# cloneofsimo/paint-with-words-sd

Measured on AMD Instinct MI355X. Metric: 512x512 images/sec (30 steps, CFG) SD1.5+PwW, higher is better.
Workload: dtype bf16

## Files before the change

__graft_entry__.py:

```python
import os
import sys

REPO = os.path.dirname(os.path.abspath(__file__))
PKG = os.path.join(REPO, "paint-with-words-sd_amd")
for p in (PKG, REPO, os.path.join(REPO, "tests")):
    if p not in sys.path:
        sys.path.insert(0, p)


def build():
    import build as pww_build
    lib = pww_build.build_lib(verbose=False)
    exe = pww_build.build_native_check()
    import pww_hip
    import paint_with_words
    handle = pww_hip.load_library()
    missing = [n for n in pww_hip.EXPORTS if not hasattr(handle, n)]
    assert not missing, "libpww_hip.so lacks %s" % missing
    from pww_hip import _lib
    built = [(lib, handle.pww_version())]
    for name, build_one in zip(pww_build.SIDE_LIBS, (pww_build.build_long, pww_build.build_scope, pww_build.build_linear, pww_build.build_regions)):
        path = build_one()
        side = _lib.load_side(name)
        assert side is not None, "%s was not built" % path
        missing = [n for n in _lib.SIDE[name]["exports"] if not hasattr(side, n)]
        assert not missing, "%s lacks %s" % (os.path.basename(path), missing)
        built.append((path, getattr(side, "pww_%s_version" % name)()))
    print("built %s and %s" % (", ".join("%s (ABI %d)" % b for b in built), exe))


def smoke():
    import math
    import numpy as np
    import torch
    import pww_hip
    from oracle import pww_oracle as O
    import pww_cases as cases

    assert torch.cuda.is_available(), "smoke() needs a HIP device"
    dev = torch.device("cuda:0")
    print("device arch:", pww_hip.device_arch())

    case = cases.make_attention_case("sd15_n1024")
    dtype = torch.float16
    mod = case["attn_cross"].to(dev, dtype)
    hidden = case["hidden"].to(dev, dtype)
    wf = lambda w, sigma, qk: 0.4 * w * math.log(1 + sigma) * qk.max()
    ctx = {"CONTEXT_TENSOR": case["ctx"].to(dev, dtype), "CROSS_ATTENTION_WEIGHT_1024": case["w"].to(dev),
           "SIGMA": torch.tensor(7.84), "WEIGHT_FUNCTION": wf}
    y = pww_hip.inj_forward(mod, hidden, ctx).float().cpu()
    mod_ref = case["attn_cross"].to("cpu", dtype).float()
    ctx_ref = {"CONTEXT_TENSOR": case["ctx"].to(dtype).float(), "CROSS_ATTENTION_WEIGHT_1024": case["w"],
               "SIGMA": torch.tensor(7.84), "WEIGHT_FUNCTION": wf}
    ref = O.inj_forward(mod_ref, case["hidden"].to(dtype).float(), ctx_ref)
    err = (y - ref).abs().max().item() / ref.abs().max().item()
    print("cross-attention + PwW bias: max err / max|O| = %.3e" % err)
    assert err < 5e-3, err

# ... 27 lines not shown
```

paint-with-words-sd_amd/build.py:

```python
import os
import subprocess
import sys

HERE = os.path.dirname(os.path.abspath(__file__))
REPO = os.path.dirname(HERE)
CSRC = os.path.join(HERE, "csrc")
LIB = os.path.join(HERE, "pww_hip", "libpww_hip.so")
LIB_EXPERIMENTS = os.path.join(HERE, "pww_hip", "libpww_hip_experiments.so")
UNITS = [("pww_api.hip", [], ""), ("pww_attn.hip", [], ""), ("pww_cross.hip", [], ""), ("pww_cross_lean.hip", [], ""), ("pww_reduce.hip", [], ""),
         ("pww_mask.hip", [], ""), ("pww_qproj.hip", [], ""), ("pww_norm.hip", [], ""), ("pww_blocks.hip", [], ""), ("pww_conv.hip", [], ""), ("pww_probs.hip", [], ""),
         ("pww_attn_inst.hip", ["-DPWW_INST_F16"], ".f16"), ("pww_attn_inst.hip", ["-DPWW_INST_BF16"], ".bf16"),
         ("pww_cross_inst.hip", ["-DPWW_INST_F16", "-DPWW_INST_NW=2"], ".f16.nw2"), ("pww_cross_inst.hip", ["-DPWW_INST_F16", "-DPWW_INST_NW=4"], ".f16.nw4"),
         ("pww_cross_inst.hip", ["-DPWW_INST_BF16", "-DPWW_INST_NW=2"], ".bf16.nw2"), ("pww_cross_inst.hip", ["-DPWW_INST_BF16", "-DPWW_INST_NW=4"], ".bf16.nw4")]
EXPERIMENT_UNITS = [("pww_cross_out.hip", [], "")]
_ATTN_HEADERS = ["pww_tile.h", "pww_attn_core.h", "pww_cross_tile.h"]
SIDE_FLAGS = ["-fvisibility=hidden"]
SIDE_LIBS = {
    "long": ("pww_long.hip", _ATTN_HEADERS, "the long-prompt launches"),
    "scope": ("pww_scope.hip", _ATTN_HEADERS, "cross-attention with per-head / per-row score statistics"),
    "linear": ("pww_linear.hip", [], "linear layers with a bias / residual / GEGLU epilogue"),
    "regions": ("pww_regions.hip", [], "region masks and the per-pixel blend of the noise predictions"),
}
SOURCES = sorted({u[0] for u in UNITS + EXPERIMENT_UNITS})
HEADERS = ["pww_common.h", "pww_tile.h", "pww_attn_core.h", "pww_attn_kernel.h", "pww_cross_tile.h", "pww_cross_kernel.h", os.path.join(REPO, "include", "pww_hip.h")]
LIB_LONG, LIB_SCOPE, LIB_LINEAR, LIB_REGIONS = (os.path.join(HERE, "pww_hip", "libpww_hip_%s.so" % n) for n in SIDE_LIBS)
LONG_UNITS, SCOPE_UNITS, LINEAR_UNITS, REGIONS_UNITS = ([(v[0], SIDE_FLAGS, "")] for v in SIDE_LIBS.values())
HIPCC = os.environ.get("HIPCC", "/opt/rocm/bin/hipcc")
FLAGS = ["--offload-arch=gfx950", "-O3", "-std=c++17", "-fPIC", "-Wall",
         "-Wno-unused-function", "-mllvm", "-amdgpu-kernarg-preload-count=16"]


PER_FILE_FLAGS = {"pww_mask.hip": ["-ffp-contract=off"], "pww_regions.hip": ["-ffp-contract=off"]}


def _newer(target, deps):
    if not os.path.exists(target):
        return True
    t = os.path.getmtime(target)
    return any(os.path.getmtime(d) > t for d in deps)


def _deps():
    return ([os.path.join(CSRC, s) for s in SOURCES] + [h if os.path.isabs(h) else os.path.join(CSRC, h) for h in HEADERS] + [__file__])


def _build(lib, units, defines, objdir, verbose, jobs=None):
    os.makedirs(objdir, exist_ok=True)
    order = sorted(units, key=lambda u: {"pww_cross_inst.hip": 0, "pww_attn_inst.hip": 1, "pww_cross_lean.hip": 2}.get(u[0], 3))
    jobs = jobs or max(2, min(len(order), os.cpu_count() or 4, int(os.environ.get("MAX_JOBS", 16))))
    pending, running, objs = list(order), [], []
    while pending or running:
        while pending and len(running) < jobs:
            src, defs, suffix = pending.pop(0)
            o = os.path.join(objdir, src + suffix + ".o")
            objs.append(o)
            cmd = [HIPCC] + FLAGS + defines + defs + PER_FILE_FLAGS.get(src, []) + ["-c", os.path.join(CSRC, src), "-o", o]
            if verbose:
                print(" ".join(cmd))
            running.append((cmd, subprocess.Popen(cmd, stdout=subprocess.PIPE, stderr=subprocess.STDOUT, text=True)))
# ... 4 lines not shown
                q.kill()
            raise RuntimeError("hipcc failed: %s\n%s" % (" ".join(cmd), out))
        if verbose and out.strip():
            print(out)
    subprocess.run([HIPCC, "--offload-arch=gfx950", "-shared", "-fPIC", "-s"] + sorted(objs) + ["-o", lib], check=True)
    return lib


def build_lib(force=False, verbose=False):
    if not force and not _newer(LIB, _deps()):
        return LIB
    return _build(LIB, UNITS, [], os.path.join(HERE, "build"), verbose)


def build_experiments(force=False, verbose=False):
    if not force and not _newer(LIB_EXPERIMENTS, _deps()):
        return LIB_EXPERIMENTS
    return _build(LIB_EXPERIMENTS, UNITS + EXPERIMENT_UNITS, ["-DPWW_EXPERIMENTS=1"], os.path.join(HERE, "build", "experiments"), verbose)


def build_side(name, force=False, verbose=False):
    unit, headers, _ = SIDE_LIBS[name]
    lib = os.path.join(HERE, "pww_hip", "libpww_hip_%s.so" % name)
    deps = [os.path.join(CSRC, f) for f in [unit, "pww_common.h", "pww_side_host.h"] + headers] + [os.path.join(REPO, "include", h) for h in ("pww_hip.h", "pww_hip_%s.h" % name)] + [__file__]
    if not force and not _newer(lib, deps):
        return lib
    return _build(lib, [(unit, SIDE_FLAGS, "")], [], os.path.join(HERE, "build", name), verbose)


def build_long(force=False, verbose=False): return build_side("long", force, verbose)
def build_scope(force=False, verbose=False): return build_side("scope", force, verbose)
def build_linear(force=False, verbose=False): return build_side("linear", force, verbose)
def build_regions(force=False, verbose=False): return build_side("regions", force, verbose)


def _build_check(exe, lib, libname, defines, force):
    src = os.path.join(REPO, "tests", "native", "attn_check.cpp")
    if not force and not _newer(exe, [src, lib, os.path.join(REPO, "include", "pww_hip.h")]):
        return exe
    cmd = [HIPCC, "--offload-arch=gfx950", "-O2", "-std=c++17"] + defines + [src, "-o", exe, "-L" + os.path.dirname(lib), "-l" + libname,
                                                                              "-Wl,-rpath,$ORIGIN/../../paint-with-words-sd_amd/pww_hip"]
    subprocess.run(cmd, check=True)
    return exe


def build_native_check(force=False):
    return _build_check(os.path.join(REPO, "tests", "native", "attn_check"), build_lib(), "pww_hip", [], force)


def build_native_check_experiments(force=False):
    return _build_check(os.path.join(REPO, "tests", "native", "attn_check_experiments"), build_experiments(), "pww_hip_experiments", ["-DPWW_EXPERIMENTS=1"], force)


if __name__ == "__main__":
    force = "--force" in sys.argv
    print(build_lib(force=force, verbose=True))
    print(build_native_check(force=force))
    for name in SIDE_LIBS:
        print(build_side(name, force=force, verbose=True))
    if "--experiments" in sys.argv:
        print(build_experiments(force=force, verbose=True))
        print(build_native_check_experiments(force=force))
```

paint-with-words-sd_amd/pww_hip/_lib.py:

```python
import ctypes
import os

_HERE = os.path.dirname(os.path.abspath(__file__))
LIB_PATH = os.environ.get("PWW_HIP_LIB", os.path.join(_HERE, "libpww_hip.so"))
EXPERIMENTS_LIB_PATH = os.environ.get("PWW_HIP_EXPERIMENTS_LIB", os.path.join(_HERE, "libpww_hip_experiments.so"))

LONG_LIB_PATH = os.environ.get("PWW_HIP_LONG_LIB", os.path.join(_HERE, "libpww_hip_long.so"))
SCOPE_LIB_PATH = os.environ.get("PWW_HIP_SCOPE_LIB", os.path.join(_HERE, "libpww_hip_scope.so"))
LINEAR_LIB_PATH = os.environ.get("PWW_HIP_LINEAR_LIB", os.path.join(_HERE, "libpww_hip_linear.so"))
REGIONS_LIB_PATH = os.environ.get("PWW_HIP_REGIONS_LIB", os.path.join(_HERE, "libpww_hip_regions.so"))

PWW_OK, PWW_EINVAL, PWW_ENOTSUP, PWW_EHIP = 0, -22, -95, -5
MIN_VERSION = 126
DTYPE_F16, DTYPE_BF16 = 0, 1
LAYOUT_NCHW, LAYOUT_NHWC = 0, 1
ACT_NONE, ACT_SILU = 0, 1
LINEAR_NONE, LINEAR_BIAS, LINEAR_BIAS_RESIDUAL, LINEAR_BIAS_GEGLU = 0, 1, 2, 3
MAX_HEAD_DIM = 160

EXPORTS = ("pww_version", "pww_has_experiments", "pww_last_error", "pww_device_arch", "pww_self_attn_fwd", "pww_cross_attn_fwd",
           "pww_cross_attn_fwd_stat", "pww_cross_attn_fwd_stat_ex",
           "pww_qk_reduce", "pww_mask_build", "pww_mask_build_rgb", "pww_mask_build_f32", "pww_resize_tokens", "pww_gauss_blur", "pww_inpaint_prep", "pww_cfg_combine", "pww_store_f32",
           "pww_workspace_bytes", "pww_profile_arm", "pww_profile_elapsed_us", "pww_profile_reset", "pww_debug_timeline", "pww_debug_path_counts",
           "pww_qproj_stat", "pww_qproj_parts", "pww_cross_attn_fwd_parts", "pww_mask_build_f32_levels", "pww_qk_parts", "pww_qk_parts_count",
           "pww_group_norm_fwd", "pww_group_norm_workspace_bytes", "pww_add_layer_norm", "pww_add_layer_norm_bias", "pww_geglu", "pww_bias_residual",
           "pww_conv3x3_workspace_bytes", "pww_conv3x3_fwd", "pww_cross_attn_probs")
EXPERIMENT_EXPORTS = ("pww_cross_attn_fwd_fused", "pww_cross_attn_fwd_fused_ex", "pww_cross_fused_workspace_bytes", "pww_cross_fused_state_bytes",
                      "pww_cross_attn_fwd_parts_out", "pww_cross_attn_out_supported")


LONG_EXPORTS = ("pww_long_version", "pww_long_last_error", "pww_long_qk_parts", "pww_long_qk_parts_count", "pww_long_cross_attn_fwd_parts",
                "pww_long_cross_attn_probs", "pww_long_profile_arm", "pww_long_profile_elapsed_us")
LONG_MIN_VERSION = 100
LONG_MIN_KEYS, LONG_MAX_KEYS = 129, 256


SCOPE_EXPORTS = ("pww_scope_version", "pww_scope_last_error", "pww_scope_head_parts_count", "pww_scope_head_parts", "pww_scope_cross_attn_fwd")
SCOPE_MIN_VERSION = 100
SCOPE_HEAD, SCOPE_ROW = 1, 2


LINEAR_EXPORTS = ("pww_linear_version", "pww_linear_last_error", "pww_linear_workspace_bytes", "pww_linear_fwd")
LINEAR_MIN_VERSION = 100


REGIONS_EXPORTS = ("pww_regions_version", "pww_regions_last_error", "pww_regions_masks", "pww_regions_combine")
REGIONS_MIN_VERSION = 100
REGIONS_MAX, REGIONS_MAX_PLANE, REGIONS_MAX_FEATHER = 8, 9216, 8.0


class AttnDesc(ctypes.Structure):
    _fields_ = [("dtype", ctypes.c_int32), ("B", ctypes.c_int32), ("H", ctypes.c_int32), ("N", ctypes.c_int32),
                ("M", ctypes.c_int32), ("D", ctypes.c_int32),
                ("q_stride", ctypes.c_int64 * 3), ("k_stride", ctypes.c_int64 * 3),
                ("v_stride", ctypes.c_int64 * 3), ("o_stride", ctypes.c_int64 * 3),
                ("scale", ctypes.c_float), ("bias_stride", ctypes.c_int64 * 4)]


class CrossOpts(ctypes.Structure):
    _fields_ = [("size", ctypes.c_uint32), ("bias_cols", ctypes.c_int32), ("coeff_scalar_dev", ctypes.c_void_p),
                ("bias_compact", ctypes.c_void_p), ("col_idx", ctypes.c_void_p), ("R", ctypes.c_int32), ("gated_images", ctypes.c_int32),
                ("compact_stride", ctypes.c_int64 * 2), ("col_idx_stride", ctypes.c_int64)]


class QprojDesc(ctypes.Structure):
    _fields_ = [("dtype", ctypes.c_int32), ("B", ctypes.c_int32), ("N", ctypes.c_int32), ("Cin", ctypes.c_int32), ("H", ctypes.c_int32),
                ("D", ctypes.c_int32), ("M", ctypes.c_int32), ("x_stride", ctypes.c_int64 * 2), ("q_stride", ctypes.c_int64 * 2),
                ("k_stride", ctypes.c_int64 * 2)]


class GnDesc(ctypes.Structure):
    _fields_ = [("dtype", ctypes.c_int32), ("layout", ctypes.c_int32), ("B", ctypes.c_int32), ("C", ctypes.c_int32), ("HW", ctypes.c_int32),
                ("G", ctypes.c_int32), ("eps", ctypes.c_float), ("act", ctypes.c_int32), ("add_stride", ctypes.c_int32), ("_pad", ctypes.c_int32)]


class LnDesc(ctypes.Structure):
    _fields_ = [("dtype", ctypes.c_int32), ("C", ctypes.c_int32), ("rows", ctypes.c_int64), ("a_stride", ctypes.c_int64), ("x_stride", ctypes.c_int64),
                ("s_stride", ctypes.c_int64), ("y_stride", ctypes.c_int64), ("eps", ctypes.c_float), ("_pad", ctypes.c_int32)]


class ConvDesc(ctypes.Structure):
    _fields_ = [("size", ctypes.c_uint32), ("dtype", ctypes.c_int32), ("B", ctypes.c_int32), ("Hin", ctypes.c_int32), ("Win", ctypes.c_int32),
                ("Cin", ctypes.c_int32), ("Cout", ctypes.c_int32), ("stride", ctypes.c_int32), ("upsample", ctypes.c_int32), ("tile_n", ctypes.c_int32),
                ("splitk", ctypes.c_int32), ("_pad", ctypes.c_int32)]


class LinearDesc(ctypes.Structure):
    _fields_ = [("size", ctypes.c_uint32), ("dtype", ctypes.c_int32), ("M", ctypes.c_int32), ("N", ctypes.c_int32), ("K", ctypes.c_int32),
                ("epilogue", ctypes.c_int32), ("x_stride", ctypes.c_int64), ("y_stride", ctypes.c_int64), ("r_stride", ctypes.c_int64),
                ("tile_n", ctypes.c_int32), ("splitk", ctypes.c_int32)]


class ProbsDesc(ctypes.Structure):
    _fields_ = [("size", ctypes.c_uint32), ("images", ctypes.c_int32), ("accumulate", ctypes.c_int32), ("weight", ctypes.c_float),
                ("out_stride", ctypes.c_int64 * 2)]


class Region(ctypes.Structure):
    _fields_ = [("r", ctypes.c_uint8), ("g", ctypes.c_uint8), ("b", ctypes.c_uint8), ("_pad", ctypes.c_uint8),
                ("strength", ctypes.c_float)]


class PwwHipError(RuntimeError):
    pass


_lib = None
_exp = None


def _bind(lib, experiments):
    vp, i32, i64, f32 = ctypes.c_void_p, ctypes.c_int32, ctypes.c_int64, ctypes.c_float
    lib.pww_version.restype = ctypes.c_int
    if lib.pww_version() // 100 != 1 or lib.pww_version() < MIN_VERSION:
        raise PwwHipError("libpww_hip ABI version %d.%02d is not 1.x >= 1.%02d (rebuild: python paint-with-words-sd_amd/build.py)"
                          % (lib.pww_version() // 100, lib.pww_version() % 100, MIN_VERSION % 100))
    lib.pww_last_error.restype = ctypes.c_char_p
# ... 104 lines not shown
    if not os.path.isfile(EXPERIMENTS_LIB_PATH):
        raise PwwHipError("libpww_hip_experiments.so not found at %s: this entry point is not part of the product library. Build it with "
                          "`python paint-with-words-sd_amd/build.py --experiments` (tests: the `experiments_lib` fixture does)." % EXPERIMENTS_LIB_PATH)
    lib = ctypes.CDLL(EXPERIMENTS_LIB_PATH)
    lib.pww_has_experiments.restype = ctypes.c_int
    if not lib.pww_has_experiments():
        raise PwwHipError("%s was not built with -DPWW_EXPERIMENTS=1" % EXPERIMENTS_LIB_PATH)
    _exp = _bind(lib, True)
    return _exp


_P = ctypes.POINTER
_vp, _i32, _i64, _f32, _f64, _sz, _int = ctypes.c_void_p, ctypes.c_int32, ctypes.c_int64, ctypes.c_float, ctypes.c_double, ctypes.c_size_t, ctypes.c_int
_HINT = "(rebuild: python paint-with-words-sd_amd/build.py, or __graft_entry__.build())"
SIDE = {
    "long": dict(path="LONG_LIB_PATH", exports=LONG_EXPORTS, min_version=LONG_MIN_VERSION, missing_ok=False, needs="prompts longer than 77 tokens need it", sigs={
        "pww_long_qk_parts": ([_vp, _vp, _vp, _P(AttnDesc), _i32, _i32, _vp, _sz, _vp], _int),
        "pww_long_qk_parts_count": ([_P(AttnDesc)], _i32),
        "pww_long_cross_attn_fwd_parts": ([_vp, _vp, _vp, _vp, _vp, _i32, _f32, _vp, _P(AttnDesc), _vp, _i32, _vp, _P(CrossOpts), _vp], _int),
        "pww_long_cross_attn_probs": ([_vp, _vp, _vp, _vp, _i32, _f64, _f32, _vp, _P(AttnDesc), _P(CrossOpts), _vp, _P(ProbsDesc), _vp], _int),
        "pww_long_profile_arm": ([], _int),
        "pww_long_profile_elapsed_us": ([_P(_f32)], _int)}),
    "scope": dict(path="SCOPE_LIB_PATH", exports=SCOPE_EXPORTS, min_version=SCOPE_MIN_VERSION, missing_ok=True, needs="per-head / per-row score statistics need it", sigs={
        "pww_scope_head_parts_count": ([_P(AttnDesc)], _i32),
        "pww_scope_head_parts": ([_vp, _vp, _vp, _P(AttnDesc), _i32, _vp, _sz, _vp], _int),
        "pww_scope_cross_attn_fwd": ([_vp, _vp, _vp, _vp, _vp, _i32, _i32, _f32, _vp, _P(AttnDesc), _vp, _i32, _vp, _P(CrossOpts), _vp], _int)}),
    "linear": dict(path="LINEAR_LIB_PATH", exports=LINEAR_EXPORTS, min_version=LINEAR_MIN_VERSION, missing_ok=False, needs="linear layers on the native kernel need it", sigs={
        "pww_linear_workspace_bytes": ([_P(LinearDesc)], _sz),
        "pww_linear_fwd": ([_vp, _vp, _vp, _vp, _vp, _P(LinearDesc), _vp, _sz, _vp], _int)}),
    "regions": dict(path="REGIONS_LIB_PATH", exports=REGIONS_EXPORTS, min_version=REGIONS_MIN_VERSION, missing_ok=False, needs="region prompts need it", sigs={
        "pww_regions_masks": ([_vp, _i32, _i32, _vp, _i32, _f32, _vp, _vp], _int),
        "pww_regions_combine": ([_vp, _vp, _vp, _vp, _f32, _vp, _i32, _i32, _i32, _i64, _i32, _vp], _int)}),
}
_side = {}


def load_side(name):
    lib = _side.get(name)
    if lib is not None:
        return lib
    spec, path, so, pre = SIDE[name], globals()[SIDE[name]["path"]], "libpww_hip_%s.so" % name, "pww_%s_" % name
    if not os.path.isfile(path):
        if spec["missing_ok"]:
            return None
        raise PwwHipError("%s not found at %s: %s %s" % (so, path, spec["needs"], _HINT))
    try:
        lib = ctypes.CDLL(path)
        getattr(lib, pre + "version").restype = _int
        version = getattr(lib, pre + "version")()
    except (OSError, AttributeError) as e:
        raise PwwHipError("%s at %s cannot be loaded: %s %s" % (so, path, e, _HINT))
    if version // 100 != 1 or version < spec["min_version"]:
        raise PwwHipError("%s ABI version %d is not 1.x >= %d %s" % (so[:-3], version, spec["min_version"], _HINT))
    missing = [n for n in spec["exports"] if not hasattr(lib, n)]
    if missing:
        raise PwwHipError("%s at %s lacks %s %s" % (so, path, missing, _HINT))
    for fn, (argtypes, restype) in spec["sigs"].items():
        getattr(lib, fn).argtypes, getattr(lib, fn).restype = argtypes, restype
    getattr(lib, pre + "last_error").restype = ctypes.c_char_p
    lib.pww_last_error = getattr(lib, pre + "last_error")
    _side[name] = lib
    return lib


def load_long():
    lib = _side.get("long")
    return lib if lib is not None else load_side("long")


def load_scope():
    lib = _side.get("scope")
    return lib if lib is not None else load_side("scope")


def load_linear():
    lib = _side.get("linear")
    return lib if lib is not None else load_side("linear")


def load_regions():
    lib = _side.get("regions")
    return lib if lib is not None else load_side("regions")


class experiments:

    def __enter__(self):
        global _lib
        load()
        self._prev = _lib
        _lib = load_experiments()
        return _lib

    def __exit__(self, *exc):
        global _lib
        _lib = self._prev
        return False


def check(rc, what, lib=None):
    if rc != PWW_OK:
        msg = (lib or load()).pww_last_error().decode("utf-8", "replace")
        raise PwwHipError("%s failed (rc=%d): %s" % (what, rc, msg))


def device_arch():
    buf = ctypes.create_string_buffer(64)
    check(load().pww_device_arch(buf, 64), "pww_device_arch")
    return buf.value.decode()
```

paint-with-words-sd_amd/pww_hip/ops.py:

```python
import ctypes

import torch

from . import _lib
from ._lib import AttnDesc, CrossOpts, ProbsDesc, QprojDesc, Region, PwwHipError

_DT = {torch.float16: _lib.DTYPE_F16, torch.bfloat16: _lib.DTYPE_BF16}


def _stream():
    return ctypes.c_void_p(torch.cuda.current_stream().cuda_stream)


def _ptr(t):
    return ctypes.c_void_p(t.data_ptr()) if t is not None else ctypes.c_void_p(0)


def _require_gpu(*tensors):
    for t in tensors:
        if t is not None and not t.is_cuda:
            raise PwwHipError("pww_hip ops need tensors on a HIP device (got %s); there is no CPU path" % t.device)


def _rows_ok(t):
    return t.stride(-1) == 1 and t.stride(0) % 8 == 0 and t.stride(1) % 8 == 0 and t.data_ptr() % 16 == 0


def _desc(q, k, v, o, heads, scale):
    if q.dim() != 3 or k.dim() != 3 or (v is not None and v.dim() != 3):
        raise PwwHipError("q/k/v must be [batch, tokens, heads*dim] tensors")
    B, N, C = q.shape
    M = k.shape[1]
    if C % heads:
# ... 869 lines not shown
    nhwc = value.is_contiguous(memory_format=torch.channels_last) and not value.is_contiguous()
    fmt = torch.channels_last if nhwc else torch.contiguous_format
    value, residual = value.contiguous(memory_format=fmt), residual.contiguous(memory_format=fmt)
    layout = _lib.LAYOUT_NHWC if nhwc else _lib.LAYOUT_NCHW
    y = torch.empty_like(value)
    with torch.cuda.device(value.device):
        _lib.check(_lib.load().pww_bias_residual(_ptr(residual), _ptr(value), _ptr(bias.contiguous()), _ptr(y), B, C, H * W, layout, _DT[value.dtype], _stream()),
                   "pww_bias_residual")
    return y


def _khwc_weight(weight):
    if weight.is_contiguous(memory_format=torch.channels_last):
        return weight
    key = (weight.data_ptr(), weight._version, weight.dtype, weight.device)
    hit = weight.__dict__.get("_pww_khwc")
    if hit is not None and hit[0] == key:
        return hit[1]
    packed = weight.detach().permute(0, 2, 3, 1).contiguous()
    weight.__dict__["_pww_khwc"] = (key, packed)
    return packed


def conv3x3_takes(x, weight, stride=1, upsample=False):
    if not (torch.is_tensor(x) and x.is_cuda and x.dim() == 4 and x.dtype in _DT and torch.is_tensor(weight) and weight.dtype == x.dtype and weight.dim() == 4):
        return False
    B, C, H, W = x.shape
    Cout = weight.shape[0]
    return (tuple(weight.shape[1:]) == (C, 3, 3) and C % 64 == 0 and Cout % 64 == 0 and stride in (1, 2) and not (upsample and stride != 1)
            and x.is_contiguous(memory_format=torch.channels_last) and x.data_ptr() % 16 == 0
            and B * H * W * C < 2 ** 31 // 4)


def conv3x3(x, weight, bias=None, residual=None, stride=1, upsample=False, tile_n=0, splitk=0):
    _require_gpu(x, weight, bias, residual)
    if not conv3x3_takes(x, weight, stride, upsample):
        raise PwwHipError("conv3x3: needs a channels_last float16/bfloat16 x with Cin, Cout multiples of 64 and a 3 x 3 weight of its dtype")
    B, C, H, W = x.shape
    Cout = weight.shape[0]
    Hv, Wv = H << int(bool(upsample)), W << int(bool(upsample))
    Ho, Wo = (Hv - 1) // stride + 1, (Wv - 1) // stride + 1
    w = _khwc_weight(weight)
    if bias is not None and (bias.dtype != x.dtype or tuple(bias.shape) != (Cout,)):
        raise PwwHipError("conv3x3: bias must be a %s [%d]" % (x.dtype, Cout))
    if bias is not None:
        bias = bias.contiguous()
    if residual is not None:
        if tuple(residual.shape) != (B, Cout, Ho, Wo) or residual.dtype != x.dtype:
            raise PwwHipError("conv3x3: residual must be a %s %s" % (x.dtype, (B, Cout, Ho, Wo)))
        residual = residual.contiguous(memory_format=torch.channels_last)
    d = _lib.ConvDesc(ctypes.sizeof(_lib.ConvDesc), _DT[x.dtype], B, H, W, C, Cout, int(stride), int(bool(upsample)), int(tile_n), int(splitk), 0)
    lib = _lib.load()
    y = torch.empty((B, Cout, Ho, Wo), dtype=x.dtype, device=x.device, memory_format=torch.channels_last)
    nbytes = int(lib.pww_conv3x3_workspace_bytes(ctypes.byref(d)))
    ws = torch.empty(nbytes // 4, dtype=torch.float32, device=x.device) if nbytes else None
    with torch.cuda.device(x.device):
        _lib.check(lib.pww_conv3x3_fwd(_ptr(x), _ptr(w), _ptr(bias), _ptr(residual), _ptr(y), ctypes.byref(d), _ptr(ws), nbytes, _stream()), "pww_conv3x3_fwd")
    return y


def _linear_weight(weight):
    if not torch.is_tensor(weight) or weight.dim() not in (2, 4) or (weight.dim() == 4 and tuple(weight.shape[2:]) != (1, 1)):
        return None
    w = weight.detach().reshape(weight.shape[0], weight.shape[1]) if weight.dim() == 4 else weight.detach()
    return w if w.is_contiguous() and w.data_ptr() == weight.data_ptr() and w.data_ptr() % 16 == 0 else None


def linear_takes(x, weight, geglu=False, bias=None, residual=None, out=None):
    if not (torch.is_tensor(x) and x.is_cuda and x.dtype in _DT and x.dim() >= 2 and torch.is_tensor(weight) and weight.dtype == x.dtype):
        return False
    w = _linear_weight(weight)
    if w is None or x.shape[-1] != w.shape[1] or x.numel() == 0 or _rows(x, "linear") is None:
        return False
    N, K = w.shape
    rows, _, xs = _rows(x, "linear")
    if not (K % 64 == 0 and N % (128 if geglu else 64) == 0 and rows * xs < 2 ** 31 and rows * N < 2 ** 31 and N * K < 2 ** 31):
        return False
    if bias is not None and not (torch.is_tensor(bias) and bias.is_cuda and bias.dtype == x.dtype and tuple(bias.shape) == (N,) and bias.is_contiguous()
                                 and bias.data_ptr() % 8 == 0):
        return False
    shape = tuple(x.shape[:-1]) + (N // 2 if geglu else N,)
    for t in (residual, out):
        if t is not None and not (torch.is_tensor(t) and t.is_cuda and t.dtype == x.dtype and tuple(t.shape) == shape and _rows(t, "linear") is not None):
            return False
    return True

# ... 42 lines not shown
```

Measured before the change: 5.111.

## Add wide-tile 3x3 conv kernel with split-K and per-shape tuned routing

Adds a new side library with a 3x3 implicit-GEMM convolution that uses larger 256x128 / 128x256 tiles over 512 threads. It double-buffers LDS with register prefetch, swizzles LDS, remaps blocks across XCDs, and does split-K with a separate fold kernel. Shapes in a tuned table (the SD1.5 UNet conv shapes at 64x64 and 32x32 latents) are routed to it by default, and the others fall back to the existing conv. The aim is better MFMA utilisation and data reuse on the large convs, at the cost of an extra fold pass and workspace traffic when split-K is used.

```diff
diff --git a/__graft_entry__.py b/__graft_entry__.py
--- a/__graft_entry__.py
+++ b/__graft_entry__.py
@@ -19,11 +19,12 @@
     assert not missing, "libpww_hip.so lacks %s" % missing
     from pww_hip import _lib
     built = [(lib, handle.pww_version())]
-    for name, build_one in zip(pww_build.SIDE_LIBS, (pww_build.build_long, pww_build.build_scope, pww_build.build_linear, pww_build.build_regions)):
+    for name, build_one in zip(pww_build.SIDE_LIBS, (pww_build.build_long, pww_build.build_scope, pww_build.build_linear, pww_build.build_regions,
+                                                     pww_build.build_conv)):
         path = build_one()
         side = _lib.load_side(name)
         assert side is not None, "%s was not built" % path
-        missing = [n for n in _lib.SIDE[name]["exports"] if not hasattr(side, n)]
+        missing = [n for n in {**_lib.SIDE, **_lib.SIDE_ROUTES}[name]["exports"] if not hasattr(side, n)]
         assert not missing, "%s lacks %s" % (os.path.basename(path), missing)
         built.append((path, getattr(side, "pww_%s_version" % name)()))
     print("built %s and %s" % (", ".join("%s (ABI %d)" % b for b in built), exe))
diff --git a/include/pww_hip_conv.h b/include/pww_hip_conv.h
--- /dev/null
+++ b/include/pww_hip_conv.h
@@ -0,0 +1,39 @@
+#ifndef PWW_HIP_CONV_H
+#define PWW_HIP_CONV_H
+
+#include "pww_hip.h"
+
+#ifdef __cplusplus
+extern "C" {
+#endif
+
+#define PWW_CONV_VERSION 100
+
+int pww_conv_version(void);
+const char *pww_conv_last_error(void);
+
+#define PWW_CONV_SCHED_AUTO 0
+#define PWW_CONV_SCHED_SHIPPED 1
+#define PWW_CONV_SCHED_SWIZZLE 2
+#define PWW_CONV_SCHED_PHASED 3
+
+typedef struct pww_conv_wide_desc {
+    uint32_t size;
+    int32_t dtype;
+    int32_t B, Hin, Win, Cin, Cout;
+    int32_t stride, upsample;
+    int32_t tile_m, tile_n, splitk;
+    int32_t schedule;
+    int32_t _pad;
+} pww_conv_wide_desc_t;
+
+int pww_conv_wide_plan(const pww_conv_wide_desc_t *desc, int32_t *tile_m, int32_t *tile_n, int32_t *split);
+size_t pww_conv_wide_workspace_bytes(const pww_conv_wide_desc_t *desc);
+int pww_conv_wide_fwd(const void *x, const void *w, const void *bias, const void *residual, void *y, const pww_conv_wide_desc_t *desc,
+                      void *workspace, size_t workspace_bytes, void *stream);
+
+#ifdef __cplusplus
+}
+#endif
+
+#endif
diff --git a/paint-with-words-sd_amd/build.py b/paint-with-words-sd_amd/build.py
--- a/paint-with-words-sd_amd/build.py
+++ b/paint-with-words-sd_amd/build.py
@@ -20,11 +20,12 @@
     "scope": ("pww_scope.hip", _ATTN_HEADERS, "cross-attention with per-head / per-row score statistics"),
     "linear": ("pww_linear.hip", [], "linear layers with a bias / residual / GEGLU epilogue"),
     "regions": ("pww_regions.hip", [], "region masks and the per-pixel blend of the noise predictions"),
+    "conv": ("pww_conv_wide.hip", [], "the 3 x 3 convolution on wide tiles"),
 }
 SOURCES = sorted({u[0] for u in UNITS + EXPERIMENT_UNITS})
 HEADERS = ["pww_common.h", "pww_tile.h", "pww_attn_core.h", "pww_attn_kernel.h", "pww_cross_tile.h", "pww_cross_kernel.h", os.path.join(REPO, "include", "pww_hip.h")]
-LIB_LONG, LIB_SCOPE, LIB_LINEAR, LIB_REGIONS = (os.path.join(HERE, "pww_hip", "libpww_hip_%s.so" % n) for n in SIDE_LIBS)
-LONG_UNITS, SCOPE_UNITS, LINEAR_UNITS, REGIONS_UNITS = ([(v[0], SIDE_FLAGS, "")] for v in SIDE_LIBS.values())
+LIB_LONG, LIB_SCOPE, LIB_LINEAR, LIB_REGIONS, LIB_CONV = (os.path.join(HERE, "pww_hip", "libpww_hip_%s.so" % n) for n in SIDE_LIBS)
+LONG_UNITS, SCOPE_UNITS, LINEAR_UNITS, REGIONS_UNITS, CONV_UNITS = ([(v[0], SIDE_FLAGS, "")] for v in SIDE_LIBS.values())
 HIPCC = os.environ.get("HIPCC", "/opt/rocm/bin/hipcc")
 FLAGS = ["--offload-arch=gfx950", "-O3", "-std=c++17", "-fPIC", "-Wall",
          "-Wno-unused-function", "-mllvm", "-amdgpu-kernarg-preload-count=16"]
@@ -95,6 +96,7 @@
 def build_scope(force=False, verbose=False): return build_side("scope", force, verbose)
 def build_linear(force=False, verbose=False): return build_side("linear", force, verbose)
 def build_regions(force=False, verbose=False): return build_side("regions", force, verbose)
+def build_conv(force=False, verbose=False): return build_side("conv", force, verbose)
 
 
 def _build_check(exe, lib, libname, defines, force):
diff --git a/paint-with-words-sd_amd/csrc/pww_conv_wide.hip b/paint-with-words-sd_amd/csrc/pww_conv_wide.hip
--- /dev/null
+++ b/paint-with-words-sd_amd/csrc/pww_conv_wide.hip
@@ -0,0 +1,361 @@
+#define PWW_SIDE_LIB "libpww_hip_conv"
+#include "pww_side_host.h"
+#include "../../include/pww_hip_conv.h"
+
+#define PWW_CONV_API extern "C" __attribute__((visibility("default")))
+
+namespace pww {
+
+namespace {
+
+constexpr int CW_THREADS = 512;
+constexpr int CW_PF = 2;
+
+__device__ __forceinline__ f32x4 mfma16(f16x8 a, f16x8 b, f32x4 c) { return __builtin_amdgcn_mfma_f32_16x16x32_f16(a, b, c, 0, 0, 0); }
+__device__ __forceinline__ f32x4 mfma16(bf16x8 a, bf16x8 b, f32x4 c) { return __builtin_amdgcn_mfma_f32_16x16x32_bf16(a, b, c, 0, 0, 0); }
+
+struct ConvCold {
+    const void *bias, *residual;
+    int nsplit, nslab;
+};
+
+__device__ __forceinline__ int xcd_remap(int orig, int nwg) {
+    const int xcd = orig & 7, q = nwg >> 3, r = nwg & 7;
+    return (xcd < r ? xcd * (q + 1) : r * (q + 1) + (xcd - r) * q) + (orig >> 3);
+}
+
+template <typename T>
+__device__ __forceinline__ void epilogue4(const f32x4 &a, const ConvCold &cold, T *y, long off, int n) {
+    typedef typename Vec<T>::v4 V4;
+    V4 o;
+#pragma unroll
+    for (int j = 0; j < 4; ++j) o[j] = (T)a[j];
+    if (cold.bias) {
+        const V4 b = *reinterpret_cast<const V4 *>(reinterpret_cast<const T *>(cold.bias) + n);
+#pragma unroll
+        for (int j = 0; j < 4; ++j) o[j] = (T)((float)o[j] + (float)b[j]);
+    }
+    if (cold.residual) {
+        const V4 r = *reinterpret_cast<const V4 *>(reinterpret_cast<const T *>(cold.residual) + off);
+#pragma unroll
+        for (int j = 0; j < 4; ++j) o[j] = (T)((float)r[j] + (float)o[j]);
+    }
+    *reinterpret_cast<V4 *>(y + off) = o;
+}
+
+template <typename T, int BM, int BN, int SCHED>
+__global__ void __launch_bounds__(CW_THREADS) __attribute__((amdgpu_waves_per_eu(2, 2))) conv3x3_wide_kernel(const T *__restrict__ x, const T *__restrict__ w, void *__restrict__ out, int M, int N,
+                                                                     int Cin, int Hin, int Win, int Wo, int HWo, const ConvCold cold) {
+    typedef typename Vec<T>::v8 V8;
+    constexpr int PF = CW_PF, XL = BM * 8 / CW_THREADS, WL = BN * 8 / CW_THREADS;
+    constexpr int WAVES_N = 8 / (BM / 64), WN = BN / WAVES_N, RM = 4, RN = WN / 16;
+    constexpr int XBYTES = BM * 128, STAGE = (BM + BN) * 128;
+    constexpr bool SWZ2 = SCHED >= PWW_CONV_SCHED_SWIZZLE, PHASED = SCHED == PWW_CONV_SCHED_PHASED;
+    __shared__ __attribute__((aligned(16))) char lds[2 * STAGE];
+
+    const int geo = cold.nslab >> 24;
+    const int nslab = cold.nslab & 0xffffff;
+    const int stride = geo & 15, up = geo >> 4;
+    const int Hv = Hin << up, Wv = Win << up;
+    const int tid = threadIdx.x, lane = tid & 63, wave = tid >> 6, wm = wave / WAVES_N, wn = wave % WAVES_N;
+    const int ntm = (M + BM - 1) / BM;
+    const int bid = xcd_remap(blockIdx.x, gridDim.x);
+    const bool split = cold.nsplit > 1;
+    const int tile = bid / cold.nsplit, ks = bid - tile * cold.nsplit;
+    const int tm = tile % ntm, tn = tile / ntm;
+    const int s_begin = (int)((long)ks * nslab / cold.nsplit), s_end = (int)((long)(ks + 1) * nslab / cold.nsplit);
+    const int K9 = 9 * Cin;
+
+    const int c = tid & 7;
+    int pix[XL], y0[XL], x0[XL];
+#pragma unroll
+    for (int i = 0; i < XL; ++i) {
+        int m = tm * BM + (tid >> 3) + 64 * i;
+        m = m < M ? m : M - 1;
+        const int b = m / HWo, rem = m - b * HWo, oy = rem / Wo, ox = rem - oy * Wo;
+        pix[i] = b * Hin * Win;
+        y0[i] = oy * stride - 1;
+        x0[i] = ox * stride - 1;
+    }
+    const T *wrow = w + (long)(tn * BN + (tid >> 3)) * K9 + c * 8;
+    const int swz = (c ^ ((SWZ2 ? tid >> 4 : tid >> 3) & 7)) << 4;
+
+    u32x4 xr[PF][XL], wr[PF][WL];
+    unsigned xok[PF];
+    int tap = s_begin / (Cin >> 6), ci0 = (s_begin - tap * (Cin >> 6)) << 6;
+    const T *wnext = wrow + s_begin * 64;
+    auto load = [&](int p) {
+        const int ky = tap / 3, kx = tap - ky * 3;
+        xok[p] = 0;
+#pragma unroll
+        for (int i = 0; i < XL; ++i) {
+            const int iyv = y0[i] + ky, ixv = x0[i] + kx;
+            const bool ok = (unsigned)iyv < (unsigned)Hv && (unsigned)ixv < (unsigned)Wv;
+            const int iy = ok ? iyv >> up : 0, ix = ok ? ixv >> up : 0;
+            xr[p][i] = *reinterpret_cast<const u32x4 *>(x + (unsigned)((pix[i] + iy * Win + ix) * Cin + ci0 + c * 8));
+            xok[p] |= (unsigned)ok << i;
+        }
+#pragma unroll
+        for (int j = 0; j < WL; ++j) wr[p][j] = *reinterpret_cast<const u32x4 *>(wnext + (long)(64 * j) * K9);
+        wnext += 64;
+        ci0 += 64;
+        if (ci0 == Cin) { ci0 = 0; ++tap; }
+    };
+    auto store_x = [&](int p, int buf) {
+        char *base = lds + buf * STAGE;
+#pragma unroll
+        for (int i = 0; i < XL; ++i) {
+            const u32x4 z = {0u, 0u, 0u, 0u};
+            *reinterpret_cast<u32x4 *>(base + ((tid >> 3) + 64 * i) * 128 + swz) = (xok[p] >> i) & 1u ? xr[p][i] : z;
+        }
+    };
+    auto store_w = [&](int p, int buf) {
+        char *base = lds + buf * STAGE + XBYTES;
+#pragma unroll
+        for (int j = 0; j < WL; ++j) *reinterpret_cast<u32x4 *>(base + ((tid >> 3) + 64 * j) * 128 + swz) = wr[p][j];
+    };
+    auto store = [&](int p, int buf) {
+        store_x(p, buf);
+        store_w(p, buf);
+    };
+
+    f32x4 acc[RN][RM];
+#pragma unroll
+    for (int r = 0; r < RN; ++r)
+#pragma unroll
+        for (int i = 0; i < RM; ++i) acc[r][i] = f32x4{0.f, 0.f, 0.f, 0.f};
+
+    const int fr = lane & 15, fq = lane >> 4;
+    auto frags = [&](int buf, int kk, V8 *xf, V8 *wf) {
+        const char *bx = lds + buf * STAGE, *bw = bx + XBYTES;
+#pragma unroll
+        for (int q = 0; q < RM; ++q) {
+            const int row = wm * 64 + q * 16 + fr;
+            xf[q] = *reinterpret_cast<const V8 *>(bx + row * 128 + (((kk * 4 + fq) ^ ((SWZ2 ? row >> 1 : row) & 7)) << 4));
+        }
+#pragma unroll
+        for (int r = 0; r < RN; ++r) {
+            const int row = wn * WN + r * 16 + fr;
+            wf[r] = *reinterpret_cast<const V8 *>(bw + row * 128 + (((kk * 4 + fq) ^ ((SWZ2 ? row >> 1 : row) & 7)) << 4));
+        }
+    };
+    auto cluster = [&](const V8 *xf, const V8 *wf) {
+#pragma unroll
+        for (int r = 0; r < RN; ++r)
+#pragma unroll
+            for (int q = 0; q < RM; ++q) acc[r][q] = mfma16(wf[r], xf[q], acc[r][q]);
+    };
+    auto slab = [&](int pl, int buf, int ps, int bufn, bool ld, bool st) {
+        if (ld) load(pl);
+        if constexpr (PHASED) {
+            V8 xf0[RM], wf0[RN], xf1[RM], wf1[RN];
+            frags(buf, 0, xf0, wf0);
+            frags(buf, 1, xf1, wf1);
+            __builtin_amdgcn_sched_barrier(0);
+            __builtin_amdgcn_s_setprio(1);
+            cluster(xf0, wf0);
+            __builtin_amdgcn_s_setprio(0);
+            __builtin_amdgcn_sched_barrier(0);
+            if (st) store_x(ps, bufn);
+            __builtin_amdgcn_sched_barrier(0);
+            __builtin_amdgcn_s_setprio(1);
+            cluster(xf1, wf1);
+            __builtin_amdgcn_s_setprio(0);
+            __builtin_amdgcn_sched_barrier(0);
+            if (st) store_w(ps, bufn);
+        } else {
+#pragma unroll
+            for (int kk = 0; kk < 2; ++kk) {
+                V8 xf[RM], wf[RN];
+                frags(buf, kk, xf, wf);
+                cluster(xf, wf);
+            }
+            if (st) store(ps, bufn);
+        }
+        __syncthreads();
+    };
+
+    const int n = s_end - s_begin;
+    load(0);
+#pragma unroll
+    for (int p = 1; p < PF; ++p)
+        if (p < n) load(p);
+    store(0, 0);
+    __syncthreads();
+    int i = 0;
+    for (; i + 2 * PF <= n; i += PF) {
+#pragma unroll
+        for (int p = 0; p < PF; ++p) slab(p, (i + p) & 1, (p + 1) % PF, (i + p + 1) & 1, true, true);
+    }
+#pragma unroll
+    for (int t = 0; t < 2 * PF - 1; ++t) {
+        if (i + t < n) slab(t % PF, (i + t) & 1, (t + 1) % PF, (i + t + 1) & 1, i + t + PF < n, i + t + 1 < n);
+    }
+
+#pragma unroll
+    for (int i = 0; i < RM; ++i) {
+        const int m = tm * BM + wm * 64 + i * 16 + fr;
+        if (m >= M) continue;
+#pragma unroll
+        for (int r = 0; r < RN; ++r) {
+            const int n = tn * BN + wn * WN + r * 16 + fq * 4;
+            if (split) *reinterpret_cast<f32x4 *>(reinterpret_cast<float *>(out) + ((long)ks * M + m) * N + n) = acc[r][i];
+            else epilogue4<T>(acc[r][i], cold, reinterpret_cast<T *>(out), (long)m * N + n, n);
+        }
+    }
+}
+
+template <typename T>
+__global__ void __launch_bounds__(256) conv3x3_wide_fold_kernel(const float *__restrict__ ws, T *__restrict__ y, long n4, int N, long MN, const ConvCold cold) {
+    const long q = (long)blockIdx.x * 256 + threadIdx.x;
+    if (q >= n4) return;
+    const long off = q * 4;
+    f32x4 a = *reinterpret_cast<const f32x4 *>(ws + off);
+    for (int s = 1; s < cold.nsplit; ++s) a += *reinterpret_cast<const f32x4 *>(ws + s * MN + off);
+    epilogue4<T>(a, cold, y, off, (int)(off % N));
+}
+
+struct ConvWideTune { int M, N, nslab, bm, bn, nsplit; };
+constexpr ConvWideTune CONV_WIDE_TUNED[] = {
+    {2048, 1280, 180, 128, 256, 3}, {2048, 640, 135, 256, 128, 6}, {2048, 640, 180, 256, 128, 6}, {2048, 640, 270, 256, 128, 6},
+    {512, 1280, 180, 128, 256, 12}, {512, 1280, 270, 128, 256, 12}, {512, 1280, 360, 128, 256, 12},
+};
+constexpr int CW_SCHED_DEFAULT = PWW_CONV_SCHED_SHIPPED;
+
+struct ConvWidePlan {
+    int M, Ho, Wo, bm, bn, nsplit, nslab, ntiles, sched;
+    bool listed;
+};
+
+bool plan_wide(const pww_conv_wide_desc_t *d, ConvWidePlan *p) {
+    if (!d || d->size < sizeof(pww_conv_wide_desc_t)) { set_error("conv_wide: descriptor missing or older than this library (size %u)", d ? d->size : 0u); return false; }
+    const int up = d->upsample, s = d->stride;
+    if ((d->dtype != PWW_DTYPE_F16 && d->dtype != PWW_DTYPE_BF16) || d->B < 1 || d->Hin < 1 || d->Win < 1 || d->Cin < 64 || d->Cin % 64 != 0
+        || d->Cout < 64 || d->Cout % 64 != 0 || (s != 1 && s != 2) || (up != 0 && up != 1) || (up && s != 1) || d->Cin > 65536 || d->Cout > 65536) {
+        set_error("conv_wide: unsupported (dtype %d B %d %dx%d Cin %d Cout %d stride %d upsample %d): Cin and Cout multiples of 64, stride 1 or 2, "
+                  "upsample only at stride 1", d->dtype, d->B, d->Hin, d->Win, d->Cin, d->Cout, s, up);
+        return false;
+    }
+    if (d->schedule < PWW_CONV_SCHED_AUTO || d->schedule > PWW_CONV_SCHED_PHASED) { set_error("conv_wide: schedule %d is not one of PWW_CONV_SCHED_*", d->schedule); return false; }
+    const int Hv = d->Hin << up, Wv = d->Win << up;
+    p->Ho = (Hv - 1) / s + 1;
+    p->Wo = (Wv - 1) / s + 1;
+    const long M = (long)d->B * p->Ho * p->Wo;
+    if ((long)d->B * d->Hin * d->Win * d->Cin >= (1L << 31) || M * d->Cout >= (1L << 31)) { set_error("conv_wide: tensor of 2^31 elements or more"); return false; }
+    p->M = (int)M;
+    p->nslab = 9 * d->Cin / 64;
+    p->sched = d->schedule ? d->schedule : CW_SCHED_DEFAULT;
+    const ConvWideTune *tuned = nullptr;
+    for (const ConvWideTune &t : CONV_WIDE_TUNED)
+        if (t.M == p->M && t.N == d->Cout && t.nslab == p->nslab) tuned = &t;
+    if (d->tile_m == 0 && d->tile_n != 0) { set_error("conv_wide: tile_n %d without tile_m", d->tile_n); return false; }
+    p->listed = d->tile_m != 0 || tuned != nullptr;
+    if (!p->listed) {
+        p->bm = p->bn = p->nsplit = p->ntiles = 0;
+        return true;
+    }
+    p->bm = d->tile_m ? d->tile_m : tuned->bm;
+    if (p->bm != 128 && p->bm != 256) { set_error("conv_wide: tile_m %d is not 128 or 256", d->tile_m); return false; }
+    p->bn = d->tile_n ? d->tile_n : d->tile_m == 0 ? tuned->bn : p->bm == 128 ? 256 : d->Cout % 128 == 0 ? 128 : 64;
+    if (!((p->bm == 256 && (p->bn == 64 || p->bn == 128)) || (p->bm == 128 && p->bn == 256))) {
+        set_error("conv_wide: no %d x %d tile (256 x 128, 256 x 64, 128 x 256)", p->bm, p->bn);
+        return false;
+    }
+    if (d->Cout % p->bn != 0) { set_error("conv_wide: tile_n %d does not divide Cout %d", p->bn, d->Cout); return false; }
+    p->ntiles = (p->M + p->bm - 1) / p->bm * (d->Cout / p->bn);
+    int ns = d->splitk;
+    if (ns <= 0 && tuned && p->bm == tuned->bm && p->bn == tuned->bn) ns = tuned->nsplit;
+    if (ns <= 0) {
+        ns = (256 + p->ntiles / 2) / p->ntiles;
+        if (ns > p->nslab / 8) ns = p->nslab / 8;
+        if (ns < 1) ns = 1;
+    }
+    if (ns > p->nslab || ns > 64) { set_error("conv_wide: split %d exceeds the %d K-slabs (or 64)", ns, p->nslab); return false; }
+    p->nsplit = ns;
+    return true;
+}
+
+template <typename T, int BM, int BN>
+void wide_launch_tile(int sched, dim3 grid, hipStream_t stream, const T *x, const T *w, void *out, int M, int N, const pww_conv_wide_desc_t *d, int Wo, int HWo,
+                      const ConvCold &cold) {
+    const dim3 block(CW_THREADS);
+    if (sched == PWW_CONV_SCHED_PHASED)
+        launch_timed(conv3x3_wide_kernel<T, BM, BN, PWW_CONV_SCHED_PHASED>, grid, block, 0, stream, x, w, out, M, N, d->Cin, d->Hin, d->Win, Wo, HWo, cold);
+    else if (sched == PWW_CONV_SCHED_SWIZZLE)
+        launch_timed(conv3x3_wide_kernel<T, BM, BN, PWW_CONV_SCHED_SWIZZLE>, grid, block, 0, stream, x, w, out, M, N, d->Cin, d->Hin, d->Win, Wo, HWo, cold);
+    else
+        launch_timed(conv3x3_wide_kernel<T, BM, BN, PWW_CONV_SCHED_SHIPPED>, grid, block, 0, stream, x, w, out, M, N, d->Cin, d->Hin, d->Win, Wo, HWo, cold);
+}
+
+template <typename T>
+int wide_launch(const ConvWidePlan &p, const pww_conv_wide_desc_t *d, const void *x, const void *w, const void *bias, const void *residual, void *y, void *ws,
+                hipStream_t stream) {
+    ConvCold cold{bias, residual, p.nsplit, p.nslab | ((d->stride | (d->upsample << 4)) << 24)};
+    const T *xt = static_cast<const T *>(x), *wt = static_cast<const T *>(w);
+    const int N = d->Cout, HWo = p.Ho * p.Wo;
+    const dim3 grid(p.ntiles * p.nsplit);
+    void *out = p.nsplit == 1 ? y : ws;
+    if (p.bm == 128) wide_launch_tile<T, 128, 256>(p.sched, grid, stream, xt, wt, out, p.M, N, d, p.Wo, HWo, cold);
+    else if (p.bn == 128) wide_launch_tile<T, 256, 128>(p.sched, grid, stream, xt, wt, out, p.M, N, d, p.Wo, HWo, cold);
+    else wide_launch_tile<T, 256, 64>(p.sched, grid, stream, xt, wt, out, p.M, N, d, p.Wo, HWo, cold);
+    if (p.nsplit == 1) return check_hip(hipGetLastError(), "conv_wide launch");
+    const long MN = (long)p.M * N, n4 = MN / 4;
+    launch_timed(conv3x3_wide_fold_kernel<T>, dim3((unsigned)((n4 + 255) / 256)), dim3(256), 0, stream, static_cast<const float *>(ws), static_cast<T *>(y),
+                 n4, N, MN, cold);
+    return check_hip(hipGetLastError(), "conv_wide fold launch");
+}
+
+size_t wide_bytes(const ConvWidePlan &p, const pww_conv_wide_desc_t *d) { return p.listed && p.nsplit > 1 ? (size_t)p.nsplit * p.M * d->Cout * sizeof(float) : 0; }
+
+}
+
+int conv_wide_plan(const pww_conv_wide_desc_t *d, int32_t *tile_m, int32_t *tile_n, int32_t *split) {
+    ConvWidePlan p;
+    if (!plan_wide(d, &p)) return PWW_ENOTSUP;
+    if (tile_m) *tile_m = p.bm;
+    if (tile_n) *tile_n = p.bn;
+    if (split) *split = p.nsplit;
+    return p.listed ? 1 : 0;
+}
+
+size_t conv_wide_workspace_bytes(const pww_conv_wide_desc_t *d) {
+    ConvWidePlan p;
+    if (!plan_wide(d, &p)) return 0;
+    return wide_bytes(p, d);
+}
+
+int conv_wide_fwd(const void *x, const void *w, const void *bias, const void *residual, void *y, const pww_conv_wide_desc_t *d, void *workspace,
+                  size_t workspace_bytes, hipStream_t stream) {
+    ConvWidePlan p;
+    if (!plan_wide(d, &p)) return PWW_ENOTSUP;
+    if (!p.listed) {
+        set_error("conv_wide: shape not listed (M %d N %d K-slabs %d) and no tile_m given: pww_conv3x3_fwd runs it", p.M, d->Cout, p.nslab);
+        return PWW_ENOTSUP;
+    }
+    if (!x || !w || !y) { set_error("conv_wide: x, w and y are required"); return PWW_EINVAL; }
+    if (!aligned16(x) || !aligned16(w) || !aligned16(y) || (reinterpret_cast<uintptr_t>(bias) & 7) || (reinterpret_cast<uintptr_t>(residual) & 7)) {
+        set_error("conv_wide: x, w, y must be 16-byte aligned, bias and residual 8-byte aligned");
+        return PWW_EINVAL;
+    }
+    const size_t need = wide_bytes(p, d);
+    if (need && (!workspace || !aligned16(workspace) || workspace_bytes < need)) {
+        set_error("conv_wide: split %d needs a 16-byte aligned workspace of %zu bytes (got %zu)", p.nsplit, need, workspace_bytes);
+        return PWW_EINVAL;
+    }
+    if (!arch_ok()) return PWW_ENOTSUP;
+    if (d->dtype == PWW_DTYPE_F16) return wide_launch<f16>(p, d, x, w, bias, residual, y, workspace, stream);
+    return wide_launch<bf16>(p, d, x, w, bias, residual, y, workspace, stream);
+}
+
+}
+
+PWW_CONV_API int pww_conv_version(void) { return PWW_CONV_VERSION; }
+PWW_CONV_API const char *pww_conv_last_error(void) { return pww::last_error(); }
+PWW_CONV_API int pww_conv_wide_plan(const pww_conv_wide_desc_t *desc, int32_t *tile_m, int32_t *tile_n, int32_t *split) {
+    return pww::conv_wide_plan(desc, tile_m, tile_n, split);
+}
+PWW_CONV_API size_t pww_conv_wide_workspace_bytes(const pww_conv_wide_desc_t *desc) { return pww::conv_wide_workspace_bytes(desc); }
+PWW_CONV_API int pww_conv_wide_fwd(const void *x, const void *w, const void *bias, const void *residual, void *y, const pww_conv_wide_desc_t *desc,
+                                   void *workspace, size_t workspace_bytes, void *stream) {
+    return pww::conv_wide_fwd(x, w, bias, residual, y, desc, workspace, workspace_bytes, static_cast<hipStream_t>(stream));
+}
diff --git a/paint-with-words-sd_amd/pww_hip/_lib.py b/paint-with-words-sd_amd/pww_hip/_lib.py
--- a/paint-with-words-sd_amd/pww_hip/_lib.py
+++ b/paint-with-words-sd_amd/pww_hip/_lib.py
@@ -9,6 +9,7 @@
 SCOPE_LIB_PATH = os.environ.get("PWW_HIP_SCOPE_LIB", os.path.join(_HERE, "libpww_hip_scope.so"))
 LINEAR_LIB_PATH = os.environ.get("PWW_HIP_LINEAR_LIB", os.path.join(_HERE, "libpww_hip_linear.so"))
 REGIONS_LIB_PATH = os.environ.get("PWW_HIP_REGIONS_LIB", os.path.join(_HERE, "libpww_hip_regions.so"))
+CONV_LIB_PATH = os.environ.get("PWW_HIP_CONV_LIB", os.path.join(_HERE, "libpww_hip_conv.so"))
 
 PWW_OK, PWW_EINVAL, PWW_ENOTSUP, PWW_EHIP = 0, -22, -95, -5
 MIN_VERSION = 126
@@ -49,6 +50,11 @@
 REGIONS_MAX, REGIONS_MAX_PLANE, REGIONS_MAX_FEATHER = 8, 9216, 8.0
 
 
+CONV_EXPORTS = ("pww_conv_version", "pww_conv_last_error", "pww_conv_wide_workspace_bytes", "pww_conv_wide_plan", "pww_conv_wide_fwd")
+CONV_MIN_VERSION = 100
+CONV_SCHED_AUTO, CONV_SCHED_SHIPPED, CONV_SCHED_SWIZZLE, CONV_SCHED_PHASED = 0, 1, 2, 3
+
+
 class AttnDesc(ctypes.Structure):
     _fields_ = [("dtype", ctypes.c_int32), ("B", ctypes.c_int32), ("H", ctypes.c_int32), ("N", ctypes.c_int32),
                 ("M", ctypes.c_int32), ("D", ctypes.c_int32),
@@ -83,6 +89,12 @@
     _fields_ = [("size", ctypes.c_uint32), ("dtype", ctypes.c_int32), ("B", ctypes.c_int32), ("Hin", ctypes.c_int32), ("Win", ctypes.c_int32),
                 ("Cin", ctypes.c_int32), ("Cout", ctypes.c_int32), ("stride", ctypes.c_int32), ("upsample", ctypes.c_int32), ("tile_n", ctypes.c_int32),
                 ("splitk", ctypes.c_int32), ("_pad", ctypes.c_int32)]
+
+
+class ConvWideDesc(ctypes.Structure):
+    _fields_ = [("size", ctypes.c_uint32), ("dtype", ctypes.c_int32), ("B", ctypes.c_int32), ("Hin", ctypes.c_int32), ("Win", ctypes.c_int32),
+                ("Cin", ctypes.c_int32), ("Cout", ctypes.c_int32), ("stride", ctypes.c_int32), ("upsample", ctypes.c_int32), ("tile_m", ctypes.c_int32),
+                ("tile_n", ctypes.c_int32), ("splitk", ctypes.c_int32), ("schedule", ctypes.c_int32), ("_pad", ctypes.c_int32)]
 
 
 class LinearDesc(ctypes.Structure):
@@ -253,6 +265,12 @@
         "pww_regions_masks": ([_vp, _i32, _i32, _vp, _i32, _f32, _vp, _vp], _int),
         "pww_regions_combine": ([_vp, _vp, _vp, _vp, _f32, _vp, _i32, _i32, _i32, _i64, _i32, _vp], _int)}),
 }
+SIDE_ROUTES = {
+    "conv": dict(path="CONV_LIB_PATH", exports=CONV_EXPORTS, min_version=CONV_MIN_VERSION, missing_ok=True, needs="the wide-tile convolution needs it", sigs={
+        "pww_conv_wide_workspace_bytes": ([_P(ConvWideDesc)], _sz),
+        "pww_conv_wide_plan": ([_P(ConvWideDesc), _P(_i32), _P(_i32), _P(_i32)], _int),
+        "pww_conv_wide_fwd": ([_vp, _vp, _vp, _vp, _vp, _P(ConvWideDesc), _vp, _sz, _vp], _int)}),
+}
 _side = {}
 
 
@@ -260,7 +278,8 @@
     lib = _side.get(name)
     if lib is not None:
         return lib
-    spec, path, so, pre = SIDE[name], globals()[SIDE[name]["path"]], "libpww_hip_%s.so" % name, "pww_%s_" % name
+    spec = SIDE[name] if name in SIDE else SIDE_ROUTES[name]
+    path, so, pre = globals()[spec["path"]], "libpww_hip_%s.so" % name, "pww_%s_" % name
     if not os.path.isfile(path):
         if spec["missing_ok"]:
             return None
@@ -304,6 +323,11 @@
     return lib if lib is not None else load_side("regions")
 
 
+def load_conv():
+    lib = _side.get("conv")
+    return lib if lib is not None else load_side("conv")
+
+
 class experiments:
 
     def __enter__(self):
diff --git a/paint-with-words-sd_amd/pww_hip/ops.py b/paint-with-words-sd_amd/pww_hip/ops.py
--- a/paint-with-words-sd_amd/pww_hip/ops.py
+++ b/paint-with-words-sd_amd/pww_hip/ops.py
@@ -1,4 +1,5 @@
 import ctypes
+import os
 
 import torch
 
@@ -934,7 +935,32 @@
             and B * H * W * C < 2 ** 31 // 4)
 
 
-def conv3x3(x, weight, bias=None, residual=None, stride=1, upsample=False, tile_n=0, splitk=0):
+def _conv_wide_route(d, tile_m, tile_n, splitk, schedule):
+    if not tile_m and (tile_n or splitk or os.environ.get("PWW_CONV_WIDE", "1") == "0"):
+        return None
+    lib = _lib.load_conv()
+    if lib is None:
+        if tile_m:
+            raise PwwHipError("conv3x3: tile_m needs libpww_hip_conv.so %s" % _lib._HINT)
+        return None
+    wd = _lib.ConvWideDesc(ctypes.sizeof(_lib.ConvWideDesc), d.dtype, d.B, d.Hin, d.Win, d.Cin, d.Cout, d.stride, d.upsample, int(tile_m), int(tile_n) if tile_m else 0,
+                           int(splitk) if tile_m else 0, int(schedule), 0)
+    if tile_m:
+        return wd
+    key = (d.dtype, d.B, d.Hin, d.Win, d.Cin, d.Cout, d.stride, d.upsample, int(schedule))
+    listed = _CONV_WIDE_LISTED.get(key)
+    if listed is None:
+        rc = lib.pww_conv_wide_plan(ctypes.byref(wd), None, None, None)
+        if rc < 0:
+            _lib.check(rc, "pww_conv_wide_plan", lib)
+        listed = _CONV_WIDE_LISTED[key] = rc == 1
+    return wd if listed else None
+
+
+_CONV_WIDE_LISTED = {}
+
+
+def conv3x3(x, weight, bias=None, residual=None, stride=1, upsample=False, tile_n=0, splitk=0, tile_m=0, schedule=0):
     _require_gpu(x, weight, bias, residual)
     if not conv3x3_takes(x, weight, stride, upsample):
         raise PwwHipError("conv3x3: needs a channels_last float16/bfloat16 x with Cin, Cout multiples of 64 and a 3 x 3 weight of its dtype")
@@ -952,8 +978,17 @@
             raise PwwHipError("conv3x3: residual must be a %s %s" % (x.dtype, (B, Cout, Ho, Wo)))
         residual = residual.contiguous(memory_format=torch.channels_last)
     d = _lib.ConvDesc(ctypes.sizeof(_lib.ConvDesc), _DT[x.dtype], B, H, W, C, Cout, int(stride), int(bool(upsample)), int(tile_n), int(splitk), 0)
+    y = torch.empty((B, Cout, Ho, Wo), dtype=x.dtype, device=x.device, memory_format=torch.channels_last)
+    wd = _conv_wide_route(d, tile_m, tile_n, splitk, schedule)
+    if wd is not None:
+        lib = _lib.load_conv()
+        nbytes = int(lib.pww_conv_wide_workspace_bytes(ctypes.byref(wd)))
+        ws = torch.empty(nbytes // 4, dtype=torch.float32, device=x.device) if nbytes else None
+        with torch.cuda.device(x.device):
+            _lib.check(lib.pww_conv_wide_fwd(_ptr(x), _ptr(w), _ptr(bias), _ptr(residual), _ptr(y), ctypes.byref(wd), _ptr(ws), nbytes, _stream()),
+                       "pww_conv_wide_fwd", lib)
+        return y
     lib = _lib.load()
-    y = torch.empty((B, Cout, Ho, Wo), dtype=x.dtype, device=x.device, memory_format=torch.channels_last)
     nbytes = int(lib.pww_conv3x3_workspace_bytes(ctypes.byref(d)))
     ws = torch.empty(nbytes // 4, dtype=torch.float32, device=x.device) if nbytes else None
     with torch.cuda.device(x.device):
```

New measurement: 5.148 (median of 6 runs). About the same (+0.7%).
